# yanxian-ll/GS-SR

Measured on AMD Instinct MI355X. Metric: train iters/sec @300k Gaussians 1080p (rasterize fwd+bwd ms and HBM GB/s vs roofline alongside), higher is better.
Workload: dtype f32; 1 GPU; diff_surfel_rasterization forward+backward (2DGS surfel: the rasterizer of configs[1] scaffold-2dgs) + fused L1/linear image loss + fused Adam (gsrast.optim, one HIP kernel) on EXPLICIT Gaussians, colors_precomp, P=300000, 1920x1080, synthetic scene SURVEY §8d (seed=rank); the complete methods (decode, SSIM, regularisers, statistics) are timed in method_iteration (--full); variant=surfel, P=300000, W=1920, H=1080, parallelism=1 independent tile(s), 1 per GPU, no collective

## Files before the change

gs-sr_amd/csrc/gsr_blend_sp.hip:

```cpp
#include "gsr_blend_common.h"
#include <hip/hip_ext.h>

#ifndef SP_WPE_EWA
#define SP_WPE_EWA 6
#endif
#ifndef SP_WPE_PLANE
#define SP_WPE_PLANE 5
#endif
#ifndef SP_WPE_SURFEL
#define SP_WPE_SURFEL 4
#endif
template <int V> struct SpOcc { static constexpr int WPE = (V == GSR_EWA) ? SP_WPE_EWA : (V == GSR_PLANE ? SP_WPE_PLANE : SP_WPE_SURFEL); };
#define SP_OCC __attribute__((amdgpu_waves_per_eu(SpOcc<V>::WPE, SpOcc<V>::WPE)))
#define SP_CH 256
#ifndef SP_CAP_EWA
#define SP_CAP_EWA 112
#endif
#ifndef SP_CAP_SURFEL
#define SP_CAP_SURFEL 111
#endif
#ifndef SP_CAP_PLANE
#define SP_CAP_PLANE 91
#endif

template <int V> struct SpTraits;
#ifndef SP_TS_PLANE
#define SP_TS_PLANE 16
#endif
#ifndef SP_NC4_EWA
#define SP_NC4_EWA 1
#endif
#ifndef SP_NC4_PLANE
#define SP_NC4_PLANE 1
#endif
template <> struct SpTraits<GSR_EWA> { static constexpr int NACC = 9, TS = 10, NREG = 10, NPIN = 9, NC4 = SP_NC4_EWA; };
template <> struct SpTraits<GSR_PLANE> { static constexpr int NACC = 16, TS = SP_TS_PLANE, NREG = 16, NPIN = 16, NC4 = SP_NC4_PLANE; };
template <> struct SpTraits<GSR_SURFEL> { static constexpr int NACC = 18, TS = 18, NREG = 21, NPIN = 21, NC4 = 1; };

__device__ __forceinline__ float row_scan_mul(float x)
{
    asm volatile("s_nop 1\n\tv_mul_f32_dpp %0, %0, %0 row_shr:1 row_mask:0xf bank_mask:0xf\n\t"
        "s_nop 1\n\tv_mul_f32_dpp %0, %0, %0 row_shr:2 row_mask:0xf bank_mask:0xf\n\t"
        "s_nop 1\n\tv_mul_f32_dpp %0, %0, %0 row_shr:4 row_mask:0xf bank_mask:0xf\n\t"
        "s_nop 1\n\tv_mul_f32_dpp %0, %0, %0 row_shr:8 row_mask:0xf bank_mask:0xf" : "+v"(x));
    return x;
}
__device__ __forceinline__ float row_scan_add(float x)
{
    asm volatile("s_nop 1\n\tv_add_f32_dpp %0, %0, %0 row_shr:1 row_mask:0xf bank_mask:0xf\n\t"
        "s_nop 1\n\tv_add_f32_dpp %0, %0, %0 row_shr:2 row_mask:0xf bank_mask:0xf\n\t"
        "s_nop 1\n\tv_add_f32_dpp %0, %0, %0 row_shr:4 row_mask:0xf bank_mask:0xf\n\t"
        "s_nop 1\n\tv_add_f32_dpp %0, %0, %0 row_shr:8 row_mask:0xf bank_mask:0xf" : "+v"(x));
    return x;
}
__device__ __forceinline__ uint32_t row_max_u32(uint32_t v)
{
#pragma unroll
    for (int d = 8; d >= 1; d >>= 1) v = max(v, (uint32_t)__shfl_xor((int)v, d, 16));
    return v;
}
__device__ __forceinline__ void lds_addf(float* p, float v) { (void)__hip_atomic_fetch_add(p, v, __ATOMIC_RELAXED, __HIP_MEMORY_SCOPE_WORKGROUP); }

template <int I> __device__ __forceinline__ float bc_mov(float c)
{
    float r;
    asm volatile("v_mov_b32_dpp %0, %1 row_newbcast:%2 row_mask:0xf bank_mask:0xf" : "=v"(r) : "v"(c), "n"(I));
    return r;
}
template <int I> __device__ __forceinline__ uint32_t bc_movu(uint32_t c)
{
    uint32_t r;
    asm volatile("v_mov_b32_dpp %0, %1 row_newbcast:%2 row_mask:0xf bank_mask:0xf" : "=v"(r) : "v"(c), "n"(I));
    return r;
}
template <int I> __device__ __forceinline__ float bc_mul(float c, float x)
{
    float r;
    asm volatile("v_mul_f32_dpp %0, %1, %2 row_newbcast:%3 row_mask:0xf bank_mask:0xf" : "=v"(r) : "v"(c), "v"(x), "n"(I));
    return r;
}
template <int I> __device__ __forceinline__ float bc_add(float c, float x)
{
    float r;
    asm volatile("v_add_f32_dpp %0, %1, %2 row_newbcast:%3 row_mask:0xf bank_mask:0xf" : "=v"(r) : "v"(c), "v"(x), "n"(I));
    return r;
}
template <int I> __device__ __forceinline__ float bc_fmac(float acc, float c, float x)
{
    asm volatile("v_fmac_f32_dpp %0, %1, %2 row_newbcast:%3 row_mask:0xf bank_mask:0xf" : "+v"(acc) : "v"(c), "v"(x), "n"(I));
    return acc;
}
template <int I> __device__ __forceinline__ float bc_fresh(float x)
{
    return __int_as_float(__builtin_amdgcn_update_dpp(0, __float_as_int(x), 0x150 + I, 0xf, 0xf, true));
}

template <int I, bool L> __device__ __forceinline__ float pc_fmac(float acc, float kc, float lc, float x) { if constexpr (L) return fmaf(lc, x, acc); else return bc_fmac<I>(acc, kc, x); }

template <int I> __device__ __forceinline__ void carry_put(float& Tc, float& Sc, float a, float b)
{
    constexpr int M = (int)~(0x00010001u << I);
    asm volatile("s_mov_b32 vcc_lo, %4\n\ts_mov_b32 vcc_hi, %4\n\ts_nop 1\n\t"
                 "v_cndmask_b32_dpp %0, %2, %0, vcc row_newbcast:15 row_mask:0xf bank_mask:0xf\n\t"
                 "v_cndmask_b32_dpp %1, %3, %1, vcc row_newbcast:15 row_mask:0xf bank_mask:0xf"
                 : "+v"(Tc), "+v"(Sc) : "v"(a), "v"(b), "n"(M) : "vcc");
}

template <int N> __device__ __forceinline__ void sp_pin(float* a)
{
    asm volatile("" : "+v"(a[0]), "+v"(a[1]), "+v"(a[2]), "+v"(a[3]), "+v"(a[4]), "+v"(a[5]), "+v"(a[6]), "+v"(a[7]), "+v"(a[8]));
    if constexpr (N > 9) asm volatile("" : "+v"(a[9]), "+v"(a[10]), "+v"(a[11]), "+v"(a[12]), "+v"(a[13]), "+v"(a[14]), "+v"(a[15]));
    if constexpr (N > 16) asm volatile("" : "+v"(a[16]), "+v"(a[17]));
    if constexpr (N > 18) asm volatile("" : "+v"(a[18]), "+v"(a[19]), "+v"(a[20]));
}

template <typename T> __device__ __forceinline__ T ld_once(const T* p) { return *p; }

template <int V> struct SpPix;
template <> struct SpPix<GSR_EWA> { float dLp0, dLp1, dLp2, Tc, Sc, rowx, rowy; uint32_t last; };
template <> struct SpPix<GSR_PLANE> { float dLp0, dLp1, dLp2, dA0, dA1, dA2, dA3, dA4, Tc, Sc, rowx, rowy; uint32_t last; };
template <> struct SpPix<GSR_SURFEL> {
    float dLp0, dLp1, dLp2, dLd, c0, c1, c2, dN0, dN1, dN2, dLmd, dMN0, dMN1, dMN2, Tc, Sc, rowx, rowy;
    uint32_t last, med;
};

struct SpSurf { float P0x, P0y, P0z, Pxx, Pxy, Pxz, Pyx, Pyy, Pyz, Tw0, Tw1, Tw2, D, cdx, cdy, oh; };
__device__ __forceinline__ SpSurf sp_surf_setup(const float4& q0, const float4& q1, const float4& q2, const float4& q4, float x0, float y0)
{
    SpSurf S;
    const float Tu0 = q0.x, Tu1 = q0.y, Tu2 = q0.z, Tv0 = q0.w, Tv1 = q1.x, Tv2 = q1.y, Tw0 = q1.z, Tw1 = q1.w, Tw2 = q2.x;
    const float kx = x0 * Tw0 - Tu0, ky = x0 * Tw1 - Tu1, kz = x0 * Tw2 - Tu2;
    const float lx = y0 * Tw0 - Tv0, ly = y0 * Tw1 - Tv1, lz = y0 * Tw2 - Tv2;
    S.P0x = ky * lz - kz * ly; S.P0y = kz * lx - kx * lz; S.P0z = kx * ly - ky * lx;
    S.Pxx = Tw1 * lz - Tw2 * ly; S.Pxy = Tw2 * lx - Tw0 * lz; S.Pxz = Tw0 * ly - Tw1 * lx;
    S.Pyx = ky * Tw2 - kz * Tw1; S.Pyy = kz * Tw0 - kx * Tw2; S.Pyz = kx * Tw1 - ky * Tw0;
    S.Tw0 = Tw0; S.Tw1 = Tw1; S.Tw2 = Tw2; S.D = q4.z;
    S.cdx = q2.y - x0; S.cdy = q2.z - y0;
    return S;
}
__device__ __forceinline__ void sp_surf_finish(const float4& t0, const float4& t1, float Tw2, float x0, float y0, const float* a , float* g )
{
    const float Tu0 = t0.x, Tu1 = t0.y, Tu2 = t0.z, Tv0 = t0.w, Tv1 = t1.x, Tv2 = t1.y, Tw0 = t1.z, Tw1 = t1.w;
    const float kx = x0 * Tw0 - Tu0, ky = x0 * Tw1 - Tu1, kz = x0 * Tw2 - Tu2;
    const float lx = y0 * Tw0 - Tv0, ly = y0 * Tw1 - Tv1, lz = y0 * Tw2 - Tv2;
    const float m0x = a[7], m0y = a[8], m0z = a[9], mxx = a[10], mxy = a[11], mxz = a[12], myx = a[13], myy = a[14], myz = a[15];
    const float ux = (m0y * lz - m0z * ly) + (myy * Tw2 - myz * Tw1);
    const float uy = (m0z * lx - m0x * lz) + (myz * Tw0 - myx * Tw2);
    const float uz = (m0x * ly - m0y * lx) + (myx * Tw1 - myy * Tw0);
    const float vx = (ky * m0z - kz * m0y) + (Tw1 * mxz - Tw2 * mxy);
    const float vy = (kz * m0x - kx * m0z) + (Tw2 * mxx - Tw0 * mxz);
    const float vz = (kx * m0y - ky * m0x) + (Tw0 * mxy - Tw1 * mxx);
    const float cx = (mxy * lz - mxz * ly) + (ky * myz - kz * myy);
    const float cy = (mxz * lx - mxx * lz) + (kz * myx - kx * myz);
    const float cz = (mxx * ly - mxy * lx) + (kx * myy - ky * myx);
    g[0] = ux; g[1] = uy; g[2] = uz; g[3] = vx; g[4] = vy; g[5] = vz;
    g[6] = a[18] - ((x0 * ux + y0 * vx) + cx);
    g[7] = a[19] - ((x0 * uy + y0 * vy) + cy);
    g[8] = a[20] - ((x0 * uz + y0 * vz) + cz);
}

template <int V, int I, int NACC>
__device__ __forceinline__ void sp_step(SpPix<V>& K, const float4* __restrict__ pcrow, const float4& q0, const float4& q1, const float4& q2, const float4& q3, const float4& q4, const SpSurf& S,
                                        bool valid, uint32_t idx0, int j, bool geo, float ddelx_dx, float ddely_dy, float* acc, uint32_t& okbits)
{
    constexpr bool L = SpTraits<V>::NC4 > 0;
    float4 pc0 = make_float4(0.f, 0.f, 0.f, 0.f);
    if constexpr (L) pc0 = pcrow[I];
    const uint32_t last = (V == GSR_EWA && L) ? __float_as_uint(pc0.w) : bc_movu<I>(K.last);
    if constexpr (V != GSR_SURFEL) {
        constexpr int DX = I & 3, DY = I >> 2;
        float dx, dy, dxx = 0.f, dxy = 0.f, dyy = 0.f, power;
        if constexpr (V == GSR_EWA) {
            dx = S.cdx - (float)DX; dy = S.cdy - (float)DY;
            dxx = dx * dx; dxy = dx * dy; dyy = dy * dy;
            power = fmaf(-0.5f, fmaf(q1.x, dyy, q0.z * dxx), -(q0.w * dxy));
        } else {
            dx = q0.x - (K.rowx + (float)DX); dy = q0.y - (K.rowy + (float)DY);
            power = -0.5f * (q0.z * dx * dx + q1.x * dy * dy) - q0.w * dx * dy;
        }
        const float G = __expf(power);
        const float alpha = fminf(0.99f, q1.y * G);
        const bool ok = valid & (idx0 < last) & !(power > 0.0f) & !(alpha < 1.0f / 255.0f);
        const float al = ok ? alpha : 0.0f, Gm = ok ? G : 0.0f;
        const float om = 1.f - al;
        const float r1a = rcp_(om);
        const float Tj = bc_fresh<I>(K.Tc) * row_scan_mul(r1a);
        const float w = al * Tj;
        float u = L ? pc0.x * q1.z : bc_mul<I>(K.dLp0, q1.z);
        u = pc_fmac<I, L>(u, K.dLp1, pc0.y, q1.w);
        u = pc_fmac<I, L>(u, K.dLp2, pc0.z, q2.x);
        if constexpr (V == GSR_PLANE) {
            if (geo) {
                u = pc_fmac<I, L>(u, K.dA0, pc0.w, q2.y); u = bc_fmac<I>(u, K.dA1, q2.z); u = bc_fmac<I>(u, K.dA2, q2.w);
                u = bc_fmac<I>(u, K.dA3, q3.x); u = bc_fmac<I>(u, K.dA4, q3.y);
            }
        }
        const float wu = w * u;
        const float si = row_scan_add(wu);
        const float Scb = bc_fresh<I>(K.Sc);
        const float Sfx = Scb + (si - wu);
        const float dL_dalpha = ok ? (u * Tj - Sfx * r1a) : 0.0f;
        carry_put<I>(K.Tc, K.Sc, Tj, Scb + si);
        acc[0] = pc_fmac<I, L>(acc[0], K.dLp0, pc0.x, w); acc[1] = pc_fmac<I, L>(acc[1], K.dLp1, pc0.y, w); acc[2] = pc_fmac<I, L>(acc[2], K.dLp2, pc0.z, w);
        if constexpr (V == GSR_EWA) {
            const float gG = Gm * dL_dalpha;
            const float h = gG * S.oh;
            acc[3] += gG;
            acc[6] = fmaf(h, dxx, acc[6]); acc[7] = fmaf(h, dxy, acc[7]); acc[8] = fmaf(h, dyy, acc[8]);
            acc[4] = fmaf(h, dx, acc[4]); acc[5] = fmaf(h, dy, acc[5]);
        } else {
            const float dL_dG = q1.y * dL_dalpha;
            const float gdx = Gm * dx, gdy = Gm * dy;
            const float dG_ddelx = -gdx * q0.z - gdy * q0.w;
            const float dG_ddely = -gdy * q1.x - gdx * q0.w;
            const float g_mx = dL_dG * dG_ddelx * ddelx_dx;
            const float g_my = dL_dG * dG_ddely * ddely_dy;
            acc[3] += Gm * dL_dalpha;
            acc[4] += g_mx; acc[5] += g_my;
            acc[6] += -0.5f * gdx * dx * dL_dG;
            acc[7] += -0.5f * gdx * dy * dL_dG;
            acc[8] += -0.5f * gdy * dy * dL_dG;
            acc[9] += fabsf(g_mx); acc[10] += fabsf(g_my);
            if (geo) {
                acc[11] = pc_fmac<I, L>(acc[11], K.dA0, pc0.w, w); acc[12] = bc_fmac<I>(acc[12], K.dA1, w); acc[13] = bc_fmac<I>(acc[13], K.dA2, w);
                acc[14] = bc_fmac<I>(acc[14], K.dA3, w); acc[15] = bc_fmac<I>(acc[15], K.dA4, w);
            }
        }
    } else {
        const float opa = q2.w;
        constexpr int DX = I & 3, DY = I >> 2;
        float ppx = S.P0x, ppy = S.P0y, ppz = S.P0z;
        if constexpr (DX != 0) { ppx = fmaf((float)DX, S.Pxx, ppx); ppy = fmaf((float)DX, S.Pxy, ppy); ppz = fmaf((float)DX, S.Pxz, ppz); }
        if constexpr (DY != 0) { ppx = fmaf((float)DY, S.Pyx, ppx); ppy = fmaf((float)DY, S.Pyy, ppy); ppz = fmaf((float)DY, S.Pyz, ppz); }
        const float rpz = (ppz == 0.0f) ? 0.0f : rcp_nr(ppz);
        const float sx = ppx * rpz, sy = ppy * rpz;
        const float rho3d = sx * sx + sy * sy;
        const float dx = S.cdx - (float)DX, dy = S.cdy - (float)DY;
        const float rho2d = FILTER_INV_SQ * (dx * dx + dy * dy);
        const float rho = fminf(rho3d, rho2d);
        const bool b3 = rho3d <= rho2d;
        const float c_d = b3 ? S.D * rpz : S.Tw2;
        const float G = __builtin_amdgcn_exp2f(rho * (-0.5f * 1.4426950408889634f));
        const float alpha = fminf(0.99f, opa * G);
        const bool ok = valid & (idx0 < last) & !(ppz == 0.0f) & !(c_d < NEAR_N) & !(alpha < 1.0f / 255.0f);
        const float al = ok ? alpha : 0.0f, cd = ok ? c_d : 1.0f;
        okbits |= ok ? (1u << I) : 0u;
        const float om = 1.f - al;
        const float r1a = rcp_(om);
        const float Tj = bc_fresh<I>(K.Tc) * row_scan_mul(r1a);
        const float w = al * Tj;
        const float rcd = rcp_(cd);
        const float m_d = fmaf(-(FAR_N * NEAR_N) / (FAR_N - NEAR_N), rcd, FAR_N / (FAR_N - NEAR_N));
        const float dmd_dd = ((FAR_N * NEAR_N) / (FAR_N - NEAR_N)) * rcd * rcd;
        float u = bc_mul<I>(K.c2, m_d * m_d);
        u = bc_fmac<I>(u, K.c1, m_d);
        u = bc_add<I>(K.c0, u);
        u = pc_fmac<I, L>(u, K.dLd, pc0.w, cd);
        u = pc_fmac<I, L>(u, K.dLp0, pc0.x, q3.w); u = pc_fmac<I, L>(u, K.dLp1, pc0.y, q4.x); u = pc_fmac<I, L>(u, K.dLp2, pc0.z, q4.y);
        u = bc_fmac<I>(u, K.dN0, q3.x); u = bc_fmac<I>(u, K.dN1, q3.y); u = bc_fmac<I>(u, K.dN2, q3.z);
        const float wu = w * u;
        const float si = row_scan_add(wu);
        const float Scb = bc_fresh<I>(K.Sc);
        const float Sfx = Scb + (si - wu);
        const float dL_dalpha = ok ? (u * Tj - Sfx * r1a) : 0.0f;
        carry_put<I>(K.Tc, K.Sc, Tj, Scb + si);
        const uint32_t med = bc_movu<I>(K.med);
        const float dLmd = bc_mov<I>(K.dLmd);
        float dL_dz = (ok & (idx0 + 1u == med)) ? dLmd : 0.0f;
        const float dL_dmd = w * bc_add<I>(K.c1, bc_mul<I>(K.c2, m_d + m_d));
        dL_dz += dL_dmd * dmd_dd;
        dL_dz = pc_fmac<I, L>(dL_dz, K.dLd, pc0.w, w);
        const float dL_dG = opa * dL_dalpha;
        const float dL_dG3 = b3 ? dL_dG : 0.0f, dL_dG2 = b3 ? 0.0f : dL_dG, dL_dz3 = b3 ? dL_dz : 0.0f;
        const float dL_dsx = dL_dG3 * -G * sx + dL_dz3 * S.Tw0;
        const float dL_dsy = dL_dG3 * -G * sy + dL_dz3 * S.Tw1;
        const float dpx = dL_dsx * rpz, dpy = dL_dsy * rpz, dpz = -(dpx * sx + dpy * sy);
        acc[0] = pc_fmac<I, L>(acc[0], K.dLp0, pc0.x, w); acc[1] = pc_fmac<I, L>(acc[1], K.dLp1, pc0.y, w); acc[2] = pc_fmac<I, L>(acc[2], K.dLp2, pc0.z, w);
        acc[3] += G * dL_dalpha;
        acc[4] = bc_fmac<I>(acc[4], K.dN0, w); acc[5] = bc_fmac<I>(acc[5], K.dN1, w); acc[6] = bc_fmac<I>(acc[6], K.dN2, w);
        acc[7] += dpx; acc[8] += dpy; acc[9] += dpz;
        if constexpr (DX != 0) { acc[10] = fmaf((float)DX, dpx, acc[10]); acc[11] = fmaf((float)DX, dpy, acc[11]); acc[12] = fmaf((float)DX, dpz, acc[12]); }
        if constexpr (DY != 0) { acc[13] = fmaf((float)DY, dpx, acc[13]); acc[14] = fmaf((float)DY, dpy, acc[14]); acc[15] = fmaf((float)DY, dpz, acc[15]); }
        acc[18] = fmaf(dL_dz3, sx, acc[18]); acc[19] = fmaf(dL_dz3, sy, acc[19]); acc[20] += dL_dz;
        acc[16] += dL_dG2 * (-G * FILTER_INV_SQ * dx);
        acc[17] += dL_dG2 * (-G * FILTER_INV_SQ * dy);
    }
}

template <int I> __device__ __forceinline__ void sp_mn_pixel(const SpPix<GSR_SURFEL>& K, uint32_t okbits, float* acc)
{
    const float okf = (float)((okbits >> I) & 1u);
    acc[4] = bc_fmac<I>(acc[4], K.dMN0, okf); acc[5] = bc_fmac<I>(acc[5], K.dMN1, okf); acc[6] = bc_fmac<I>(acc[6], K.dMN2, okf);
}

template <int V> __device__ __attribute__((noinline)) uint32_t sp_quadrant_mask_slow(const float4* __restrict__ cull, uint32_t id, int tx, int ty)
{
    const float4 ca = cull[2 * (size_t)id], cb = cull[2 * (size_t)id + 1];
    uint32_t m = 0;
#pragma unroll
    for (int q = 0; q < 4; q++)
        if (cull_hit_rec<V>(ca, cb, (float)(tx * GSR_TILE + (q & 1) * GSR_SUB), (float)(ty * GSR_TILE + (q >> 1) * GSR_SUB), 7.f)) m |= 1u << q;
    return m;
}

template <int V>
__global__ void __launch_bounds__(256) SP_OCC k_blend_bwd_sp(BlendParams p)
{
    using TR = SpTraits<V>;
    constexpr int ST = (V == GSR_EWA) ? GSR_REC_EWA : (V == GSR_PLANE ? GSR_REC_PLANE : GSR_REC_SURFEL);
    constexpr int AS = (V == GSR_EWA) ? GSR_ACC_EWA : (V == GSR_PLANE ? GSR_ACC_PLANE : GSR_ACC_SURFEL);
    constexpr int NACC = TR::NACC, TS = TR::TS, NREG = TR::NREG;

    constexpr int CAPV = (V == GSR_EWA) ? SP_CAP_EWA : (V == GSR_PLANE ? SP_CAP_PLANE : SP_CAP_SURFEL);
    __shared__ float2 s_wtab[4 * CAPV * (TS / 2)];
    __shared__ uint8_t s_cidx[4 * SP_CH];
    __shared__ uint32_t s_ids[SP_CH];
    __shared__ uint32_t s_lo[4];
    __shared__ uint16_t s_mask[SP_CH];
    __shared__ uint8_t s_cent[4 * CAPV];
    __shared__ uint8_t s_queue[4 * 4 * CAPV];
    __shared__ uint32_t s_wmax[4];
    constexpr int NC4 = TR::NC4;
    constexpr int PCW = 64, PCR = 16;
    __shared__ float4 s_pc[NC4 > 0 ? 4 * PCW * NC4 : 1];

    const int tile = tile_of_block(blockIdx.x, p.gx * p.gy, p.tile_order, p.static_map);
    const int tx = tile % p.gx, ty = tile / p.gx;
    const int wave = threadIdx.x >> 6, lane = threadIdx.x & 63;
    const int b = lane >> 4, j = lane & 15;
    const int qx = tx * GSR_TILE + (wave & 1) * GSR_SUB, qy = ty * GSR_TILE + (wave >> 1) * GSR_SUB;
    const int px = qx + (b & 1) * 4 + (j & 3), py = qy + (b >> 1) * 4 + (j >> 2);
    const bool inside = px < p.W && py < p.H;
    const uint2 range = p.ranges[tile];
    const size_t HW = (size_t)p.W * p.H;
    const uint32_t pix_id = inside ? (uint32_t)p.W * py + px : 0u;

    SpPix<V> K;
    const float T_final = inside ? ld_once(p.final_T + pix_id) : 0.f;
    K.last = inside ? ld_once(p.n_contrib + pix_id) : 0u;
    K.dLp0 = K.dLp1 = K.dLp2 = 0.f;
    if (inside && p.dL_dcolor) { K.dLp0 = ld_once(p.dL_dcolor + pix_id); K.dLp1 = ld_once(p.dL_dcolor + HW + pix_id); K.dLp2 = ld_once(p.dL_dcolor + 2 * HW + pix_id); }
    K.rowx = (float)(qx + (b & 1) * 4); K.rowy = (float)(qy + (b >> 1) * 4);
    K.Tc = T_final;
    K.Sc = T_final * (p.bg[0] * K.dLp0 + p.bg[1] * K.dLp1 + p.bg[2] * K.dLp2);
    const bool geo = (V == GSR_PLANE) && p.render_geo;
    if constexpr (V == GSR_PLANE) {
        float dA[5] = { 0, 0, 0, 0, 0 };
        if (geo && inside) {
            const float rayx = (float)(((float)px - p.W * 0.5) / p.fx), rayy = (float)(((float)py - p.H * 0.5) / p.fy);
            if (p.dL_dout_all_map)
                for (int c = 0; c < 5; c++) dA[c] = ld_once(p.dL_dout_all_map + c * HW + pix_id);
            const float nx = ld_once(p.all_map_pixels + pix_id), ny = ld_once(p.all_map_pixels + HW + pix_id), nz = ld_once(p.all_map_pixels + 2 * HW + pix_id);
            const float distance = ld_once(p.all_map_pixels + 4 * HW + pix_id);
            const float tmp = (float)(nx * rayx + ny * rayy + nz + 1.0e-8);
            const float dpd = p.dL_dplane_depth ? ld_once(p.dL_dplane_depth + pix_id) : 0.f;
            dA[4] += (-dpd / tmp);
            dA[0] += dpd * (distance / (tmp * tmp) * rayx);
            dA[1] += dpd * (distance / (tmp * tmp) * rayy);
            dA[2] += dpd * (distance / (tmp * tmp));
        }
        K.dA0 = dA[0]; K.dA1 = dA[1]; K.dA2 = dA[2]; K.dA3 = dA[3]; K.dA4 = dA[4];
    }
    if constexpr (V == GSR_SURFEL) {
        K.dLd = K.c0 = K.c1 = K.c2 = K.dN0 = K.dN1 = K.dN2 = K.dLmd = K.dMN0 = K.dMN1 = K.dMN2 = 0.f;
        K.med = 0;
        if (inside) {
            float dLa = 0.f, dLr = 0.f;
            K.med = ld_once(p.n_contrib + pix_id + HW);
            if (p.dL_dothers) {
                const float* g = p.dL_dothers;
                K.dLd = ld_once(g + 0 * HW + pix_id); dLa = ld_once(g + 1 * HW + pix_id); K.dN0 = ld_once(g + 2 * HW + pix_id); K.dN1 = ld_once(g + 3 * HW + pix_id); K.dN2 = ld_once(g + 4 * HW + pix_id);
                K.dLmd = ld_once(g + 5 * HW + pix_id); dLr = ld_once(g + 6 * HW + pix_id); K.dMN0 = ld_once(g + 8 * HW + pix_id); K.dMN1 = ld_once(g + 9 * HW + pix_id); K.dMN2 = ld_once(g + 10 * HW + pix_id);
            }
            const float fD = ld_once(p.final_T + pix_id + HW), fD2 = ld_once(p.final_T + pix_id + 2 * HW);
            K.c0 = fmaf(dLr, fD2, dLa); K.c1 = -2.0f * dLr * fD; K.c2 = dLr * (1.f - T_final);
        }
    }
    if constexpr (V == GSR_SURFEL) s_pc[wave * PCW + b * PCR + j] = make_float4(K.dLp0, K.dLp1, K.dLp2, K.dLd);
    if constexpr (V == GSR_EWA && NC4 > 0) s_pc[wave * PCW + b * PCR + j] = make_float4(K.dLp0, K.dLp1, K.dLp2, __uint_as_float(K.last));
    if constexpr (V == GSR_PLANE && NC4 > 0) s_pc[wave * PCW + b * PCR + j] = make_float4(K.dLp0, K.dLp1, K.dLp2, K.dA0);
    const float4* pcrow = s_pc + (NC4 > 0 ? wave * PCW + b * PCR : 0);
    bool mn_live = false;
    if constexpr (V == GSR_SURFEL) mn_live = __ballot((K.dMN0 != 0.f) | (K.dMN1 != 0.f) | (K.dMN2 != 0.f)) != 0ull;
    const uint32_t mlast_row = row_max_u32(K.last);
    uint32_t mlast_b[4];
#pragma unroll
    for (int k = 0; k < 4; k++) mlast_b[k] = (uint32_t)__builtin_amdgcn_readlane((int)mlast_row, 16 * k);
    const uint32_t wmax = max(max(mlast_b[0], mlast_b[1]), max(mlast_b[2], mlast_b[3]));
    if (lane == 0) s_wmax[wave] = wmax;
    __syncthreads();
    const uint32_t tile_max = max(max(s_wmax[0], s_wmax[1]), max(s_wmax[2], s_wmax[3]));
    if (tile_max == 0) return;

    const uint8_t* myqueue = s_queue + (wave * 4 + b) * CAPV;
    const float ddelx_dx = 0.5f * p.W, ddely_dy = 0.5f * p.H;

    float2* mytab = s_wtab + wave * CAPV * (TS / 2);
    uint8_t* mycidx = s_cidx + wave * SP_CH;
    uint8_t* mycent = s_cent + wave * CAPV;
    uint32_t hi = tile_max;
    while (hi > 0) {
        const uint32_t n = min((uint32_t)SP_CH, hi);
        const uint32_t cbase = hi - n;
        {
            const uint32_t t = threadIdx.x;
            if (t < n) {
                const uint32_t id = p.point_list[range.x + cbase + t];
                s_ids[t] = id;
                uint32_t m = 0;
                if (p.qmask) {
                    const uint32_t ei = cbase + t;
                    const unsigned long long* q = p.qmask + (((size_t)(range.x >> 6) + (size_t)tile + (ei >> 6)) << 2);
#pragma unroll
                    for (int w4 = 0; w4 < 4; w4++) m |= (uint32_t)((q[w4] >> (ei & 63u)) & 1ull) << w4;
                } else m = sp_quadrant_mask_slow<V>(p.cull, id, tx, ty);
                s_mask[t] = (uint16_t)m;
            }
        }
        __syncthreads();
        {
            uint32_t run = 0, first = 0;
            for (int e0 = (int)((n - 1u) & ~63u); e0 >= 0; e0 -= 64) {
                const uint32_t e = (uint32_t)e0 + lane;
                uint64_t am = __ballot((e < n) && (((uint32_t)s_mask[e] >> wave) & 1u) && (cbase + e < wmax));
                const uint32_t c = (uint32_t)__popcll(am);
                if (run + c > (uint32_t)CAPV) {
                    while ((uint32_t)__popcll(am) > (uint32_t)CAPV - run) am &= am - 1ull;
                    first = (uint32_t)e0 + (am ? (uint32_t)__ffsll((unsigned long long)am) - 1u : 64u);
                    break;
                }
                run += c;
            }
            if (lane == 0) s_lo[wave] = first;
        }
        __syncthreads();
        const uint32_t lo_e = max(max(s_lo[0], s_lo[1]), max(s_lo[2], s_lo[3]));
        uint32_t cany = 0;
        for (uint32_t e0 = 0; e0 < n; e0 += 64) {
            const uint32_t e = e0 + lane;
            const bool any = (e >= lo_e) && (e < n) && (((uint32_t)s_mask[e] >> wave) & 1u) && (cbase + e < wmax);
            const uint64_t am = __ballot(any);
            const uint32_t arank = __builtin_amdgcn_mbcnt_hi((uint32_t)(am >> 32), __builtin_amdgcn_mbcnt_lo((uint32_t)am, 0u));
            if (e < n) mycidx[e] = any ? (uint8_t)min(cany + arank, 255u) : (uint8_t)0xFF;
            if (any && cany + arank < CAPV) mycent[cany + arank] = (uint8_t)e;
            cany += (uint32_t)__popcll(am);
        }
        uint32_t cnt[4] = { 0, 0, 0, 0 };
        for (uint32_t i0 = 0; i0 < min(cany, (uint32_t)CAPV); i0 += 64) {
            const uint32_t i = i0 + lane;
            const bool v = i < min(cany, (uint32_t)CAPV);
            const uint32_t e = v ? (uint32_t)mycent[i] : 0u;
            const uint32_t id = s_ids[e];
            float4 ca = make_float4(0.f, 0.f, 0.f, 0.f), cb = make_float4(0.f, -1.f, 0.f, 0.f);
            if (v) { ca = p.cull[2 * (size_t)id]; cb = p.cull[2 * (size_t)id + 1]; }
            const uint32_t hit4 = cull_hit_quad4<V>(ca, cb, (float)qx, (float)qy);
#pragma unroll
            for (int k = 0; k < 4; k++) {
                const bool hit = v && (cbase + e < mlast_b[k]) && ((hit4 >> k) & 1u);
                const uint64_t bm = __ballot(hit);
                const uint32_t rank = __builtin_amdgcn_mbcnt_hi((uint32_t)(bm >> 32), __builtin_amdgcn_mbcnt_lo((uint32_t)bm, 0u));
                if (hit) s_queue[(wave * 4 + k) * CAPV + cnt[k] + rank] = (uint8_t)e;
                cnt[k] += (uint32_t)__popcll(bm);
            }
        }
        for (uint32_t q = lane; q < cany * (TS / 2); q += 64) mytab[q] = make_float2(0.f, 0.f);
        const int Qmine = (int)(b == 0 ? cnt[0] : (b == 1 ? cnt[1] : (b == 2 ? cnt[2] : cnt[3])));
        const int loads = (int)((max(max(cnt[0], cnt[1]), max(cnt[2], cnt[3])) + 15u) >> 4);

#ifdef SP_DIAG_NO_LOADS
        for (int ld = 0; ld < 0; ld++) {
#else
        for (int ld = 0; ld < loads; ld++) {
#endif
            const int pos = Qmine - 1 - (16 * ld + j);
            const bool valid = pos >= 0;
            const uint32_t e = valid ? (uint32_t)myqueue[pos] : 0u;
            const uint32_t gid = s_ids[e];
            const uint32_t idx0 = cbase + e;
            const float4* __restrict__ r = p.rec + (size_t)gid * ST;
            const float4 z4 = make_float4(0.f, 0.f, 0.f, 0.f);
            const float4 q0 = valid ? r[0] : z4, q1 = valid ? r[1] : z4, q2 = valid ? r[2] : z4;
            float4 q3 = z4, q4 = z4;
            if (V != GSR_EWA) q3 = valid ? r[3] : z4;
            if (V == GSR_SURFEL) q4 = valid ? r[4] : z4;
            float acc[NREG];
#pragma unroll
            for (int c = 0; c < NREG; c++) acc[c] = 0.f;
            SpSurf S = {};
            uint32_t okbits = 0u;
            if constexpr (V == GSR_SURFEL) S = sp_surf_setup(q0, q1, q2, q4, K.rowx, K.rowy);
            else if constexpr (V == GSR_EWA) { S.cdx = q0.x - K.rowx; S.cdy = q0.y - K.rowy; S.oh = -0.5f * q1.y; }
            const bool never = p.gx == 0x7fffffff;
#define SP_STEP(I) sp_step<V, I, NACC>(K, pcrow, q0, q1, q2, q3, q4, S, valid, idx0, j, geo, ddelx_dx, ddely_dy, acc, okbits); sp_pin<TR::NPIN>(acc); if (never) asm volatile("s_nop 0");
#ifndef SP_DIAG_NO_STEPS
            SP_STEP(0) SP_STEP(1) SP_STEP(2) SP_STEP(3) SP_STEP(4) SP_STEP(5) SP_STEP(6) SP_STEP(7)
            SP_STEP(8) SP_STEP(9) SP_STEP(10) SP_STEP(11)
#endif
            float4 t0 = z4, t1 = z4;
            if constexpr (V == GSR_SURFEL) { t0 = r[0]; t1 = r[1]; }
#ifndef SP_DIAG_NO_STEPS
            SP_STEP(12) SP_STEP(13) SP_STEP(14) SP_STEP(15)
#endif
#undef SP_STEP
            if constexpr (V == GSR_EWA) {
                const float sx = acc[4], sy = acc[5];
                acc[4] = (2.0f * ddelx_dx) * fmaf(q0.w, sy, q0.z * sx);
                acc[5] = (2.0f * ddely_dy) * fmaf(q0.w, sx, q1.x * sy);
            }
            if constexpr (V == GSR_SURFEL) {
                if (mn_live) {
#define SP_MN(I) sp_mn_pixel<I>(K, okbits, acc);
                    SP_MN(0) SP_MN(1) SP_MN(2) SP_MN(3) SP_MN(4) SP_MN(5) SP_MN(6) SP_MN(7) SP_MN(8) SP_MN(9) SP_MN(10) SP_MN(11) SP_MN(12) SP_MN(13) SP_MN(14) SP_MN(15)
#undef SP_MN
                }
                float g9[9];
                sp_surf_finish(t0, t1, S.Tw2, K.rowx, K.rowy, acc, g9);
#pragma unroll
                for (int c = 0; c < 9; c++) acc[7 + c] = g9[c];
            }
            const uint32_t cid = valid ? (uint32_t)mycidx[e] : 0u;
#pragma unroll
            for (int rr = 0; rr < 4; rr++) {
                if (b == rr && valid) {
                    float2* t = mytab + cid * (TS / 2);
#pragma unroll
                    for (int c = 0; c < (NACC + 1) / 2; c++) { float2 v = t[c]; v.x += acc[2 * c]; v.y += acc[2 * c + 1]; t[c] = v; }
                }
            }
        }
        __syncthreads();
        for (uint32_t e = lo_e + (threadIdx.x >> 4); e < n; e += 16) {
            const uint32_t c = threadIdx.x & 15u;
            float v0 = 0.f, v1 = 0.f;
#pragma unroll
            for (int w = 0; w < 4; w++) {
                const uint32_t ci = s_cidx[w * SP_CH + e];
                if (ci != 0xFFu) {
                    const float* t = reinterpret_cast<const float*>(s_wtab + (w * CAPV + ci) * (TS / 2));
                    if ((int)c < NACC) v0 += t[c];
                    if (NACC > 16 && (int)c < NACC - 16) v1 += t[16 + c];
                }
            }
            float* dst = p.acc + (size_t)s_ids[e] * AS;
#ifndef SP_DIAG_NO_FLUSH
            if (v0 != 0.f) atomic_addf(dst + c, v0);
            if (NACC > 16 && v1 != 0.f) atomic_addf(dst + 16 + c, v1);
#else
            if (v0 == 123.456f && v1 == 1.f) dst[c] = v0;
#endif
        }
        hi = cbase + lo_e;
        if (hi > 0) __syncthreads();
    }
}

static thread_local hipEvent_t t_ev_start = nullptr, t_ev_stop = nullptr;
void gsr_blend_bwd_attach_events(hipEvent_t start, hipEvent_t stop) { t_ev_start = start; t_ev_stop = stop; }

int gsr_launch_blend_bwd_sp(const BlendParams& p, int variant, hipStream_t s)
{
    dim3 grid(p.gx * p.gy), block(256);
    if (t_ev_start && t_ev_stop) {
        hipEvent_t a = t_ev_start, b = t_ev_stop;
        t_ev_start = t_ev_stop = nullptr;
        switch (variant) {
        case GSR_EWA: hipExtLaunchKernelGGL(k_blend_bwd_sp<GSR_EWA>, grid, block, 0, s, a, b, 0, p); break;
        case GSR_PLANE: hipExtLaunchKernelGGL(k_blend_bwd_sp<GSR_PLANE>, grid, block, 0, s, a, b, 0, p); break;
        default: hipExtLaunchKernelGGL(k_blend_bwd_sp<GSR_SURFEL>, grid, block, 0, s, a, b, 0, p); break;
        }
        return 0;
    }
    switch (variant) {
    case GSR_EWA: hipLaunchKernelGGL(k_blend_bwd_sp<GSR_EWA>, grid, block, 0, s, p); break;
    case GSR_PLANE: hipLaunchKernelGGL(k_blend_bwd_sp<GSR_PLANE>, grid, block, 0, s, p); break;
    default: hipLaunchKernelGGL(k_blend_bwd_sp<GSR_SURFEL>, grid, block, 0, s, p); break;
    }
    return 0;
}
```

Measured before the change: 1403 iters/s.

## Decouple backward blend quadrant waves into independent per-wave workgroups

Restructures the splat backward blend so each quadrant wave works on its own, with its own chunk table and id/position rows, using wave-level barriers instead of block-wide __syncthreads. For surfel and plane the launch becomes one 64-thread workgroup per quadrant (4x grid); EWA keeps four waves per group. Chunking now follows each wave's own last-contributor bound and quadrant mask bits instead of a shared tile chunk, and the per-wave tables are flushed without the cross-wave reduction. This removes block-level barriers and lets quadrants finish independently, in exchange for more atomics per Gaussian, since the four quadrants no longer merge before flushing, and more workgroups.

```diff
diff --git a/gs-sr_amd/csrc/gsr_blend_sp.hip b/gs-sr_amd/csrc/gsr_blend_sp.hip
--- a/gs-sr_amd/csrc/gsr_blend_sp.hip
+++ b/gs-sr_amd/csrc/gsr_blend_sp.hip
@@ -10,17 +10,29 @@
 #ifndef SP_WPE_SURFEL
 #define SP_WPE_SURFEL 4
 #endif
-template <int V> struct SpOcc { static constexpr int WPE = (V == GSR_EWA) ? SP_WPE_EWA : (V == GSR_PLANE ? SP_WPE_PLANE : SP_WPE_SURFEL); };
+#ifndef SP_WPG_EWA
+#define SP_WPG_EWA 4
+#endif
+#ifndef SP_WPG_PLANE
+#define SP_WPG_PLANE 1
+#endif
+#ifndef SP_WPG_SURFEL
+#define SP_WPG_SURFEL 1
+#endif
+template <int V> struct SpOcc {
+    static constexpr int WPE = (V == GSR_EWA) ? SP_WPE_EWA : (V == GSR_PLANE ? SP_WPE_PLANE : SP_WPE_SURFEL);
+    static constexpr int WPG = (V == GSR_EWA) ? SP_WPG_EWA : (V == GSR_PLANE ? SP_WPG_PLANE : SP_WPG_SURFEL);
+};
 #define SP_OCC __attribute__((amdgpu_waves_per_eu(SpOcc<V>::WPE, SpOcc<V>::WPE)))
-#define SP_CH 256
+#define SP_SPAN 65535u
 #ifndef SP_CAP_EWA
-#define SP_CAP_EWA 112
+#define SP_CAP_EWA 107
 #endif
 #ifndef SP_CAP_SURFEL
-#define SP_CAP_SURFEL 111
+#define SP_CAP_SURFEL 112
 #endif
 #ifndef SP_CAP_PLANE
-#define SP_CAP_PLANE 91
+#define SP_CAP_PLANE 89
 #endif
 
 template <int V> struct SpTraits;
@@ -303,8 +315,15 @@
     return m;
 }
 
+__device__ __forceinline__ void sp_wave_sync()
+{
+    __builtin_amdgcn_fence(__ATOMIC_RELEASE, "wavefront");
+    __builtin_amdgcn_wave_barrier();
+    __builtin_amdgcn_fence(__ATOMIC_ACQUIRE, "wavefront");
+}
+
 template <int V>
-__global__ void __launch_bounds__(256) SP_OCC k_blend_bwd_sp(BlendParams p)
+__global__ void __launch_bounds__(64 * SpOcc<V>::WPG) SP_OCC k_blend_bwd_sp(BlendParams p)
 {
     using TR = SpTraits<V>;
     constexpr int ST = (V == GSR_EWA) ? GSR_REC_EWA : (V == GSR_PLANE ? GSR_REC_PLANE : GSR_REC_SURFEL);
@@ -312,23 +331,36 @@
     constexpr int NACC = TR::NACC, TS = TR::TS, NREG = TR::NREG;
 
     constexpr int CAPV = (V == GSR_EWA) ? SP_CAP_EWA : (V == GSR_PLANE ? SP_CAP_PLANE : SP_CAP_SURFEL);
-    __shared__ float2 s_wtab[4 * CAPV * (TS / 2)];
-    __shared__ uint8_t s_cidx[4 * SP_CH];
-    __shared__ uint32_t s_ids[SP_CH];
-    __shared__ uint32_t s_lo[4];
-    __shared__ uint16_t s_mask[SP_CH];
-    __shared__ uint8_t s_cent[4 * CAPV];
-    __shared__ uint8_t s_queue[4 * 4 * CAPV];
-    __shared__ uint32_t s_wmax[4];
+    static_assert(CAPV >= 64 && CAPV <= 256, "a 64-entry batch must fit an empty table; the queues hold a table row in one byte");
     constexpr int NC4 = TR::NC4;
-    constexpr int PCW = 64, PCR = 16;
-    __shared__ float4 s_pc[NC4 > 0 ? 4 * PCW * NC4 : 1];
-
-    const int tile = tile_of_block(blockIdx.x, p.gx * p.gy, p.tile_order, p.static_map);
+    constexpr int WPG = SpOcc<V>::WPG;
+    constexpr int PCR = 16, PCW = NC4 > 0 ? 64 * NC4 : 1;
+    __shared__ float4 g_pc[WPG * PCW];
+    __shared__ float2 g_tab[WPG * CAPV * (TS / 2)];
+    __shared__ uint32_t g_rid[WPG * CAPV];
+    __shared__ uint16_t g_rpos[WPG * CAPV];
+    __shared__ uint8_t g_queue[WPG * 4 * CAPV];
+    const int wgw = (WPG > 1) ? __builtin_amdgcn_readfirstlane((int)(threadIdx.x >> 6)) : 0, lane = threadIdx.x & 63;
+    float4* const s_pc = g_pc + wgw * PCW;
+    float2* const s_tab = g_tab + wgw * CAPV * (TS / 2);
+    uint32_t* const s_rid = g_rid + wgw * CAPV;
+    uint16_t* const s_rpos = g_rpos + wgw * CAPV;
+    uint8_t* const s_queue = g_queue + wgw * 4 * CAPV;
+
+    constexpr int QPG = 4 / WPG;
+    int tb, wave;
+    {
+        const int T = p.gx * p.gy, w = (int)blockIdx.x, full = (T >> 3) * 8 * QPG;
+        int h;
+        if (w < full) { const int m = w >> 3; h = m % QPG; tb = ((m / QPG) << 3) + (w & 7); }
+        else { const int r = w - full, R = T & 7; h = r / R; tb = (T & ~7) + r % R; }
+        wave = h * WPG + wgw;
+    }
+    const int tile = tile_of_block(tb, p.gx * p.gy, p.tile_order, p.static_map);
     const int tx = tile % p.gx, ty = tile / p.gx;
-    const int wave = threadIdx.x >> 6, lane = threadIdx.x & 63;
     const int b = lane >> 4, j = lane & 15;
     const int qx = tx * GSR_TILE + (wave & 1) * GSR_SUB, qy = ty * GSR_TILE + (wave >> 1) * GSR_SUB;
+    if (qx >= p.W || qy >= p.H) return;
     const int px = qx + (b & 1) * 4 + (j & 3), py = qy + (b >> 1) * 4 + (j >> 2);
     const bool inside = px < p.W && py < p.H;
     const uint2 range = p.ranges[tile];
@@ -376,10 +408,10 @@
             K.c0 = fmaf(dLr, fD2, dLa); K.c1 = -2.0f * dLr * fD; K.c2 = dLr * (1.f - T_final);
         }
     }
-    if constexpr (V == GSR_SURFEL) s_pc[wave * PCW + b * PCR + j] = make_float4(K.dLp0, K.dLp1, K.dLp2, K.dLd);
-    if constexpr (V == GSR_EWA && NC4 > 0) s_pc[wave * PCW + b * PCR + j] = make_float4(K.dLp0, K.dLp1, K.dLp2, __uint_as_float(K.last));
-    if constexpr (V == GSR_PLANE && NC4 > 0) s_pc[wave * PCW + b * PCR + j] = make_float4(K.dLp0, K.dLp1, K.dLp2, K.dA0);
-    const float4* pcrow = s_pc + (NC4 > 0 ? wave * PCW + b * PCR : 0);
+    if constexpr (V == GSR_SURFEL) s_pc[b * PCR + j] = make_float4(K.dLp0, K.dLp1, K.dLp2, K.dLd);
+    if constexpr (V == GSR_EWA && NC4 > 0) s_pc[b * PCR + j] = make_float4(K.dLp0, K.dLp1, K.dLp2, __uint_as_float(K.last));
+    if constexpr (V == GSR_PLANE && NC4 > 0) s_pc[b * PCR + j] = make_float4(K.dLp0, K.dLp1, K.dLp2, K.dA0);
+    const float4* pcrow = s_pc + (NC4 > 0 ? b * PCR : 0);
     bool mn_live = false;
     if constexpr (V == GSR_SURFEL) mn_live = __ballot((K.dMN0 != 0.f) | (K.dMN1 != 0.f) | (K.dMN2 != 0.f)) != 0ull;
     const uint32_t mlast_row = row_max_u32(K.last);
@@ -387,83 +419,77 @@
 #pragma unroll
     for (int k = 0; k < 4; k++) mlast_b[k] = (uint32_t)__builtin_amdgcn_readlane((int)mlast_row, 16 * k);
     const uint32_t wmax = max(max(mlast_b[0], mlast_b[1]), max(mlast_b[2], mlast_b[3]));
-    if (lane == 0) s_wmax[wave] = wmax;
-    __syncthreads();
-    const uint32_t tile_max = max(max(s_wmax[0], s_wmax[1]), max(s_wmax[2], s_wmax[3]));
-    if (tile_max == 0) return;
-
-    const uint8_t* myqueue = s_queue + (wave * 4 + b) * CAPV;
+    if (wmax == 0) return;
+    sp_wave_sync();
+
+    const uint8_t* myqueue = s_queue + b * CAPV;
     const float ddelx_dx = 0.5f * p.W, ddely_dy = 0.5f * p.H;
 
-    float2* mytab = s_wtab + wave * CAPV * (TS / 2);
-    uint8_t* mycidx = s_cidx + wave * SP_CH;
-    uint8_t* mycent = s_cent + wave * CAPV;
-    uint32_t hi = tile_max;
+    const unsigned long long* qw = p.qmask ? p.qmask + ((((size_t)(range.x >> 6) + (size_t)tile) << 2) + wave) : nullptr;
+    uint32_t hi = wmax;
     while (hi > 0) {
-        const uint32_t n = min((uint32_t)SP_CH, hi);
-        const uint32_t cbase = hi - n;
-        {
-            const uint32_t t = threadIdx.x;
-            if (t < n) {
-                const uint32_t id = p.point_list[range.x + cbase + t];
-                s_ids[t] = id;
-                uint32_t m = 0;
-                if (p.qmask) {
-                    const uint32_t ei = cbase + t;
-                    const unsigned long long* q = p.qmask + (((size_t)(range.x >> 6) + (size_t)tile + (ei >> 6)) << 2);
-#pragma unroll
-                    for (int w4 = 0; w4 < 4; w4++) m |= (uint32_t)((q[w4] >> (ei & 63u)) & 1ull) << w4;
-                } else m = sp_quadrant_mask_slow<V>(p.cull, id, tx, ty);
-                s_mask[t] = (uint16_t)m;
-            }
-        }
-        __syncthreads();
-        {
-            uint32_t run = 0, first = 0;
-            for (int e0 = (int)((n - 1u) & ~63u); e0 >= 0; e0 -= 64) {
-                const uint32_t e = (uint32_t)e0 + lane;
-                uint64_t am = __ballot((e < n) && (((uint32_t)s_mask[e] >> wave) & 1u) && (cbase + e < wmax));
-                const uint32_t c = (uint32_t)__popcll(am);
-                if (run + c > (uint32_t)CAPV) {
-                    while ((uint32_t)__popcll(am) > (uint32_t)CAPV - run) am &= am - 1ull;
-                    first = (uint32_t)e0 + (am ? (uint32_t)__ffsll((unsigned long long)am) - 1u : 64u);
-                    break;
+        uint32_t ln = (uint32_t)lane;
+        asm volatile("" : "+v"(ln));
+        uint32_t run = 0, lo = 0;
+        uint32_t wv_lo = 0, wv_hi = 0;
+        int wtop = -1;
+        for (int bi = (int)((hi - 1u) >> 6); bi >= 0; bi--) {
+            if (hi - 1u - ((uint32_t)bi << 6) > SP_SPAN) { lo = ((uint32_t)bi + 1u) << 6; break; }
+            const uint32_t pos = ((uint32_t)bi << 6) + ln;
+            uint64_t am;
+            if (qw) {
+                if (wtop < 0 || bi < wtop - 63) {
+                    wtop = bi;
+                    const unsigned long long w = ((uint32_t)bi >= ln) ? qw[(size_t)((uint32_t)bi - ln) << 2] : 0ull;
+                    wv_lo = (uint32_t)w; wv_hi = (uint32_t)(w >> 32);
                 }
-                run += c;
-            }
-            if (lane == 0) s_lo[wave] = first;
-        }
-        __syncthreads();
-        const uint32_t lo_e = max(max(s_lo[0], s_lo[1]), max(s_lo[2], s_lo[3]));
-        uint32_t cany = 0;
-        for (uint32_t e0 = 0; e0 < n; e0 += 64) {
-            const uint32_t e = e0 + lane;
-            const bool any = (e >= lo_e) && (e < n) && (((uint32_t)s_mask[e] >> wave) & 1u) && (cbase + e < wmax);
-            const uint64_t am = __ballot(any);
-            const uint32_t arank = __builtin_amdgcn_mbcnt_hi((uint32_t)(am >> 32), __builtin_amdgcn_mbcnt_lo((uint32_t)am, 0u));
-            if (e < n) mycidx[e] = any ? (uint8_t)min(cany + arank, 255u) : (uint8_t)0xFF;
-            if (any && cany + arank < CAPV) mycent[cany + arank] = (uint8_t)e;
-            cany += (uint32_t)__popcll(am);
-        }
+                const int k = wtop - bi;
+                am = ((uint64_t)(uint32_t)__builtin_amdgcn_readlane((int)wv_hi, k) << 32) | (uint32_t)__builtin_amdgcn_readlane((int)wv_lo, k);
+            } else {
+                bool h = false;
+                if (pos < range.y - range.x) h = (sp_quadrant_mask_slow<V>(p.cull, p.point_list[range.x + pos], tx, ty) >> wave) & 1u;
+                am = __ballot(h);
+            }
+            if ((((uint32_t)bi + 1u) << 6) > hi) am &= (1ull << (hi & 63u)) - 1ull;
+            uint32_t c = (uint32_t)__popcll(am);
+            const bool full = run + c > (uint32_t)CAPV;
+            if (full) {
+                while ((uint32_t)__popcll(am) > (uint32_t)CAPV - run) am &= am - 1ull;
+                c = (uint32_t)CAPV - run;
+                lo = ((uint32_t)bi << 6) + (am ? (uint32_t)__ffsll((unsigned long long)am) - 1u : 64u);
+            }
+            if ((am >> ln) & 1ull) {
+                const uint32_t rank = __builtin_amdgcn_mbcnt_hi((uint32_t)(am >> 32), __builtin_amdgcn_mbcnt_lo((uint32_t)am, 0u));
+                const uint32_t row = (uint32_t)CAPV - run - c + rank;
+                s_rid[row] = p.point_list[range.x + pos];
+                s_rpos[row] = (uint16_t)(hi - 1u - pos);
+            }
+            run += c;
+            if (full) break;
+        }
+        const uint32_t first = (uint32_t)CAPV - run;
+        sp_wave_sync();
         uint32_t cnt[4] = { 0, 0, 0, 0 };
-        for (uint32_t i0 = 0; i0 < min(cany, (uint32_t)CAPV); i0 += 64) {
-            const uint32_t i = i0 + lane;
-            const bool v = i < min(cany, (uint32_t)CAPV);
-            const uint32_t e = v ? (uint32_t)mycent[i] : 0u;
-            const uint32_t id = s_ids[e];
+        for (uint32_t i0 = 0; i0 < run; i0 += 64) {
+            const uint32_t i = i0 + ln;
+            const bool v = i < run;
+            const uint32_t row = v ? first + i : (uint32_t)CAPV - 1u;
+            const uint32_t id = s_rid[row];
+            const uint32_t lpos = hi - 1u - (uint32_t)s_rpos[row];
             float4 ca = make_float4(0.f, 0.f, 0.f, 0.f), cb = make_float4(0.f, -1.f, 0.f, 0.f);
             if (v) { ca = p.cull[2 * (size_t)id]; cb = p.cull[2 * (size_t)id + 1]; }
             const uint32_t hit4 = cull_hit_quad4<V>(ca, cb, (float)qx, (float)qy);
 #pragma unroll
             for (int k = 0; k < 4; k++) {
-                const bool hit = v && (cbase + e < mlast_b[k]) && ((hit4 >> k) & 1u);
+                const bool hit = v && (lpos < mlast_b[k]) && ((hit4 >> k) & 1u);
                 const uint64_t bm = __ballot(hit);
                 const uint32_t rank = __builtin_amdgcn_mbcnt_hi((uint32_t)(bm >> 32), __builtin_amdgcn_mbcnt_lo((uint32_t)bm, 0u));
-                if (hit) s_queue[(wave * 4 + k) * CAPV + cnt[k] + rank] = (uint8_t)e;
+                if (hit) s_queue[k * CAPV + cnt[k] + rank] = (uint8_t)row;
                 cnt[k] += (uint32_t)__popcll(bm);
             }
         }
-        for (uint32_t q = lane; q < cany * (TS / 2); q += 64) mytab[q] = make_float2(0.f, 0.f);
+        for (uint32_t q = ln; q < run * (TS / 2); q += 64) s_tab[first * (TS / 2) + q] = make_float2(0.f, 0.f);
+        sp_wave_sync();
         const int Qmine = (int)(b == 0 ? cnt[0] : (b == 1 ? cnt[1] : (b == 2 ? cnt[2] : cnt[3])));
         const int loads = (int)((max(max(cnt[0], cnt[1]), max(cnt[2], cnt[3])) + 15u) >> 4);
 
@@ -474,9 +500,9 @@
 #endif
             const int pos = Qmine - 1 - (16 * ld + j);
             const bool valid = pos >= 0;
-            const uint32_t e = valid ? (uint32_t)myqueue[pos] : 0u;
-            const uint32_t gid = s_ids[e];
-            const uint32_t idx0 = cbase + e;
+            const uint32_t cid = valid ? (uint32_t)myqueue[pos] : (uint32_t)CAPV - 1u;
+            const uint32_t gid = s_rid[cid];
+            const uint32_t idx0 = hi - 1u - (uint32_t)s_rpos[cid];
             const float4* __restrict__ r = p.rec + (size_t)gid * ST;
             const float4 z4 = make_float4(0.f, 0.f, 0.f, 0.f);
             const float4 q0 = valid ? r[0] : z4, q1 = valid ? r[1] : z4, q2 = valid ? r[2] : z4;
@@ -518,30 +544,23 @@
 #pragma unroll
                 for (int c = 0; c < 9; c++) acc[7 + c] = g9[c];
             }
-            const uint32_t cid = valid ? (uint32_t)mycidx[e] : 0u;
 #pragma unroll
             for (int rr = 0; rr < 4; rr++) {
                 if (b == rr && valid) {
-                    float2* t = mytab + cid * (TS / 2);
+                    float2* t = s_tab + cid * (TS / 2);
 #pragma unroll
                     for (int c = 0; c < (NACC + 1) / 2; c++) { float2 v = t[c]; v.x += acc[2 * c]; v.y += acc[2 * c + 1]; t[c] = v; }
                 }
             }
         }
-        __syncthreads();
-        for (uint32_t e = lo_e + (threadIdx.x >> 4); e < n; e += 16) {
-            const uint32_t c = threadIdx.x & 15u;
+        sp_wave_sync();
+        for (uint32_t row = first + (uint32_t)b; row < (uint32_t)CAPV; row += 4) {
+            const uint32_t c = (uint32_t)j;
+            const float* t = reinterpret_cast<const float*>(s_tab + row * (TS / 2));
             float v0 = 0.f, v1 = 0.f;
-#pragma unroll
-            for (int w = 0; w < 4; w++) {
-                const uint32_t ci = s_cidx[w * SP_CH + e];
-                if (ci != 0xFFu) {
-                    const float* t = reinterpret_cast<const float*>(s_wtab + (w * CAPV + ci) * (TS / 2));
-                    if ((int)c < NACC) v0 += t[c];
-                    if (NACC > 16 && (int)c < NACC - 16) v1 += t[16 + c];
-                }
-            }
-            float* dst = p.acc + (size_t)s_ids[e] * AS;
+            if ((int)c < NACC) v0 = t[c];
+            if (NACC > 16 && (int)c < NACC - 16) v1 = t[16 + c];
+            float* dst = p.acc + (size_t)s_rid[row] * AS;
 #ifndef SP_DIAG_NO_FLUSH
             if (v0 != 0.f) atomic_addf(dst + c, v0);
             if (NACC > 16 && v1 != 0.f) atomic_addf(dst + 16 + c, v1);
@@ -549,8 +568,8 @@
             if (v0 == 123.456f && v1 == 1.f) dst[c] = v0;
 #endif
         }
-        hi = cbase + lo_e;
-        if (hi > 0) __syncthreads();
+        hi = lo;
+        sp_wave_sync();
     }
 }
 
@@ -559,7 +578,8 @@
 
 int gsr_launch_blend_bwd_sp(const BlendParams& p, int variant, hipStream_t s)
 {
-    dim3 grid(p.gx * p.gy), block(256);
+    const int wpg = variant == GSR_EWA ? SpOcc<GSR_EWA>::WPG : (variant == GSR_PLANE ? SpOcc<GSR_PLANE>::WPG : SpOcc<GSR_SURFEL>::WPG);
+    dim3 grid((4 / wpg) * p.gx * p.gy), block(64 * wpg);
     if (t_ev_start && t_ev_stop) {
         hipEvent_t a = t_ev_start, b = t_ev_stop;
         t_ev_start = t_ev_stop = nullptr;
```

Result: no change. 1431 iters/s (median of 5 runs) (+2.0%).
